# bing164/PL-VI-ORBSLAM3

Hardware: AMD Instinct MI355X
Metric: frames/sec ORB+LSD extract+match, 640×480 mono, 1/2/4/8 MI355X (higher is better)
Workload: dtype u8; 1 GPU; C1+C2+C3: ORB extract (1000 feats, 1.2, 8 levels, FAST 20/7) || LSD+LBD (200 lines, scale 0.8, 2 octaves) as one HIP-stream schedule, then ORB kNN-2 + LineMatcher::match vs previous frame; batch=3072, width=640, height=480, parallelism=sequence-sharded x1, gather=False, inflight=2

## Files before the change

### include/plvi_frontend.h

```cpp
#ifndef PLVI_FRONTEND_H
#define PLVI_FRONTEND_H

#include <stddef.h>
#include <stdint.h>

#ifdef __cplusplus
extern "C" {
#endif

enum {
  PLVI_OK = 0,
  PLVI_E_EMPTY = -1,
  PLVI_E_BADARG = -2,
  PLVI_E_CAPACITY = -3,
  PLVI_E_HIP = -4,
  PLVI_E_OVERFLOW = -5,
  PLVI_E_SIZE = -6,
  PLVI_E_CAPTURE = -7,
};

enum {
  PLVI_COMPAT_GAUSS_ROUNDED = 1,
  PLVI_COMPAT_RESIZE_V_GENERIC = 2,
  PLVI_COMPAT_EXP_CV_TABLE = 4,
// ... 90 lines not shown
int plvi_lines_extract_batch(plvi_line_extractor* h, const uint8_t* d_frames, int n_frames, size_t frame_stride,
                             size_t row_stride, void* stream);
int plvi_lines_outputs(plvi_line_extractor* h, plvi_keyline** d_kl, uint8_t** d_desc, double** d_fn, int** d_count,
                       int* cap);
int plvi_lines_errors(plvi_line_extractor* h, int* frame_flags, int* any, void* stream);

int plvi_lines_pyramid_level(plvi_line_extractor* h, int frame, int level, uint8_t* dst, int* w, int* hgt);

int plvi_lines_scale_tables(plvi_line_extractor* h, float* scale, float* inv_scale, float* sigma2, float* inv_sigma2);

int plvi_lines_profile(plvi_line_extractor* h, int enable);
int plvi_lines_debug_stats(plvi_line_extractor* h, unsigned long long* d_stats);
int plvi_lines_debug_mw_stats(plvi_line_extractor* h, int* d_stats);
int plvi_lines_debug_planes(plvi_line_extractor* h, int frame, int octave, float* deg, double* modgrad, float* cs,
                            int* sw, int* sh);
int plvi_lines_debug_sobel(plvi_line_extractor* h, int frame, int octave, short* dxdy, int* w, int* hgt);
int plvi_lines_debug_raw_lines(plvi_line_extractor* h, int frame, int octave, float* out, int cap, int* n);
int plvi_lines_profile_read(plvi_line_extractor* h, float* stage_ms, int* runs);
int plvi_lines_kernel_timing(plvi_line_extractor* h, int enable);
int plvi_lines_kernel_timing_read(plvi_line_extractor* h, float* total_ms, int* launches);
int plvi_lines_kernel_timing_read_kind(plvi_line_extractor* h, int kind, float* total_ms, int* launches);


int plvi_hamming_knn2_batch(const uint8_t* d_q, const int* d_nq, int nq_cap, const uint8_t* d_t, const int* d_nt,
                            int nt_cap, int n_pairs, int* d_idx0, int* d_d0, int* d_idx1, int* d_d1, void* stream);

int plvi_hamming_knn2(const uint8_t* q, int nq, const uint8_t* t, int nt, int* idx0, int* d0, int* idx1, int* d1);

int plvi_line_match_nnr(const uint8_t* desc1, int n1, const uint8_t* desc2, int n2, float nnr, int* matches_12);

// ... 756 lines not shown
```

### pl-vi-orbslam3_amd/csrc/lines_kernels.hpp

```cpp
#include <hip/hip_runtime.h>

#include "block_prims.h"
#include "lines_device.h"
#include "plvi_common.h"
#include "plvi_math.h"
#include "std_sort.h"

namespace plvi {

constexpr double kNotdef = -1024.0;
constexpr float kNotdefF = -1024.0f;
constexpr double kD2R = 3.14159265358979323846 / 180;
constexpr double kPi = 3.14159265358979323846;
constexpr double kLog10Of11 = 0x1.0a98b6050c56fp+0;

__global__ __launch_bounds__(256) void lsd_half_kernel(const uint8_t* __restrict__ src, size_t s_frame, size_t s_row,
                                                       uint8_t* __restrict__ dst, int dw, int dh, size_t d_frame) {
    const int f = blockIdx.y;
    const int i = blockIdx.x * 256 + threadIdx.x;
    if (i >= dw * dh) return;
    const int y = i / dw, x = i % dw;
    const uint8_t* S0 = src + (size_t)f * s_frame + (size_t)(2 * y) * s_row;
    const uint8_t* S1 = S0 + s_row;
    const int s = S0[2 * x] + S0[2 * x + 1] + S1[2 * x] + S1[2 * x + 1];
// ... 183 lines not shown
__device__ __forceinline__ void vm_drain() { __builtin_amdgcn_s_waitcnt(0); }

__device__ __forceinline__ bool used_get(const GrowCtx& g, int x, int y) {
    const bool inwin = y < g.wbb + g.RB;
    const int yy = inwin ? y : g.wbb;
    unsigned v = g.bits[(yy & (g.RB - 1)) * g.wpr + (x >> 5)];
    if (__builtin_expect(!inwin, 0)) v = gload_l2(g.gbits + (size_t)y * g.wpr + (x >> 5));
    return y < g.ys || ((v >> (x & 31)) & 1u);
}
__device__ __forceinline__ void used_set(const GrowCtx& g, int x, int y) {
    const unsigned b = 1u << (x & 31);
    if (__builtin_expect(y < g.wbb + g.RB, 1))
        __atomic_fetch_or(&g.bits[(y & (g.RB - 1)) * g.wpr + (x >> 5)], b, __ATOMIC_RELAXED);
    else __hip_atomic_fetch_or(g.gbits + (size_t)y * g.wpr + (x >> 5), b, __ATOMIC_RELAXED, __HIP_MEMORY_SCOPE_AGENT);
}
__device__ __forceinline__ void used_set_chunk(const GrowCtx& g, int xb, int y, unsigned long long mask, int lane) {
    const unsigned w = lane == 0 ? (unsigned)mask : (unsigned)(mask >> 32);
    if (lane < 2 && w) __atomic_fetch_or(&g.bits[(y & (g.RB - 1)) * g.wpr + (xb >> 5) + lane], w, __ATOMIC_RELAXED);
    __builtin_amdgcn_wave_barrier();
    __builtin_amdgcn_fence(__ATOMIC_ACQ_REL, "wavefront");
}
__device__ __forceinline__ unsigned q_get(const GrowCtx& g, int i) {
    if (__builtin_expect(i < g.QL, 1)) return g.qlds[i];
    return gload_l2(g.qglob + (i - g.QL));
}
__device__ __forceinline__ void q_put(const GrowCtx& g, int i, unsigned v) {
    if (__builtin_expect(i < g.QL, 1)) g.qlds[i] = v;
    else gstore_l2(g.qglob + (i - g.QL), v);
}
__device__ __forceinline__ float deg_at(const GrowCtx& g, int x, int y) {
    if (g.R == 0) return g.P[(size_t)y * g.sw + x];
    const bool inwin = y < g.wb + g.R;
    const int yy = inwin ? y : g.wb;
    float v = g.win[(yy & (g.R - 1)) * g.sw + x];
    if (__builtin_expect(!inwin, 0)) v = g.P[(size_t)y * g.sw + x];
    return v;
// ... 43 lines not shown
        }
    }
    for (; i < n; i += 64) {
        const int row = r0 + i / g.sw, x = i % g.sw;
        g.win[(row & (g.R - 1)) * g.sw + x] = src[i];
    }
}
__device__ __forceinline__ void bits_load_rows(const GrowCtx& g, int r0, int r1, int lane) {
    const int nw = (r1 - r0) * g.wpr;
    for (int k = lane; k < nw; k += 64) {
        const int row = r0 + k / g.wpr, w = k % g.wpr;
        g.bits[(row & (g.RB - 1)) * g.wpr + w] = gload_l2(g.gbits + (size_t)row * g.wpr + w);
    }
}

#ifndef PLVI_GROW_SETPRIO
#define PLVI_GROW_SETPRIO 3
#endif
#ifndef PLVI_GROW_OCT1_PRIO
#define PLVI_GROW_OCT1_PRIO PLVI_GROW_SETPRIO
#endif

#ifndef PLVI_GROW_WPE
#define PLVI_GROW_WPE 8
#endif
#ifndef PLVI_GROW_WG_WAVES
#define PLVI_GROW_WG_WAVES 4
#endif
constexpr int kGrowWaves = PLVI_GROW_WG_WAVES;

__device__ __forceinline__ void grow_wave_sync() {
    __builtin_amdgcn_fence(__ATOMIC_RELEASE, "wavefront");
    __builtin_amdgcn_wave_barrier();
    __builtin_amdgcn_fence(__ATOMIC_ACQUIRE, "wavefront");
    __builtin_amdgcn_sched_barrier(0);
}

constexpr int kGrowRB = 64, kGrowQL = 256;

template <bool STATS, bool FIXED, bool LOOP = false>
__global__ __launch_bounds__(64 * kGrowWaves, PLVI_GROW_WPE) void lsd_grow_kernel(const LineOctDev* __restrict__ octs,
                                                      const float* __restrict__ pix,
                                                      const double* __restrict__ modgrad,
                                                      const float2* __restrict__ pixcs,
                                                      unsigned* __restrict__ gbits_all, size_t gbits_frame,
                                                      unsigned* __restrict__ qspill, size_t qspill_frame,
                                                      double prec, LsdRegion* __restrict__ regs, unsigned* __restrict__ regpts,
                                                      size_t regpts_frame, int* __restrict__ nlines,
                                                      int* __restrict__ err, int R, int RB, int QL, int nOct,
                                                      int oBase, int oCount, unsigned long long* __restrict__ stats,
                                                      int nf, int ldsWave, int wpw) {
    extern __shared__ __align__(16) unsigned lds_all[];
    __builtin_amdgcn_s_setprio(PLVI_GROW_SETPRIO);
    const int wv = __builtin_amdgcn_readfirstlane((int)(threadIdx.x >> 6));
    const int ntask = nf * oCount, tstride = LOOP ? (int)gridDim.x * wpw : ntask;
    for (int task0 = blockIdx.x * wpw + wv; task0 < ntask; task0 += tstride) {
    const int task = __builtin_amdgcn_readfirstlane(task0);
    const int o = oBase + task / nf, f = task - (o - oBase) * nf;
    if (PLVI_GROW_OCT1_PRIO != PLVI_GROW_SETPRIO && o > 0) __builtin_amdgcn_s_setprio(PLVI_GROW_OCT1_PRIO);
    lds_u32* lds_w = (lds_u32*)lds_all + wv * (ldsWave >> 2);
// ... 3 lines not shown
    GrowCtx g;
    if (FIXED) {
        R = 0;
        RB = kGrowRB;
        QL = kGrowQL;
    }
    g.sw = sw; g.sh = sh; g.R = R; g.RB = RB; g.QL = QL;
    g.wpr = (sw + 31) >> 5;
    g.P = pix + od.soff + (size_t)f * od.splane;
    const float2* SC = pixcs + od.soff + (size_t)f * od.splane;
    LsdRegion* outR = regs + (size_t)(f * nOct + o) * kLsdRawCap;
    unsigned* outP = regpts + (size_t)(f * nOct + o) * regpts_frame;
    int npts = 0;
    g.gbits = gbits_all + (size_t)(f * nOct + o) * gbits_frame;
    g.qglob = qspill + (size_t)(f * nOct + o) * qspill_frame;
    g.bits = lds_w;
    g.qlds = g.bits + RB * g.wpr;
    g.win = (lds_f32*)(g.qlds + QL);
    g.wb = 0;
    g.wbb = 0;
    g.ys = 0;
    for (int i = lane; i < sh * g.wpr; i += 64) g.gbits[i] = 0u;
    for (int i = lane; i < RB * g.wpr; i += 64) g.bits[i] = 0u;
    if (R) win_load_rows(g, 0, min(R, sh), lane);
    vm_drain();
    grow_wave_sync();
    int nout = 0;
    bool overflow = false;
    const float pdeg = (float)(prec / kD2R);
    const int min_reg = od.min_reg_size;
    const int bp = lane / 9, bk = lane % 9;
    const int kdx = bk % 3 - 1, kdy = bk / 3 - 1;
    const unsigned long long below = (1ull << lane) - 1ull;
    unsigned long long s_setup = 0, s_round = 0, s_rect = 0, n_seed = 0, n_block = 0, n_round = 0, n_rpt = 0,
                       n_commit = 0;
    unsigned long long s_ph[4] = {0, 0, 0, 0};
    unsigned long long s_scan = 0, s_seed = 0, s_init = 0;
    unsigned long long n_far = 0, n_spill = 0;
    constexpr bool do_stats = STATS;
    const unsigned long long t_begin = do_stats ? __builtin_amdgcn_s_memtime() : 0;
    unsigned long long t_mark = t_begin;
    const unsigned long long t_real0 = do_stats ? __builtin_amdgcn_s_memrealtime() : 0;
    const int half = R / 2, halfb = RB / 2;
    auto chunk_load = [&](int cy, int cxb, float* v) {
        const int x = cxb + lane, xm = max(x - 1, 0), xx = min(x, sw - 1), xp = min(x + 1, sw - 1);
        const float* r0 = g.P + (size_t)cy * sw;
        const float* r1 = r0 + sw;
        v[0] = r0[xx]; v[1] = r0[xm]; v[2] = r0[xp];
        v[3] = r1[xm]; v[4] = r1[xx]; v[5] = r1[xp];
    };
    auto chunk_next = [&](int& cy, int& cxb) {
        if (cxb + 64 < sw - 1) {
            cxb += 64;
        } else {
            cxb = 0;
            ++cy;
        }
    };
    float nv[6], nv2[6];
    int py2 = 0, px2 = 0;
    chunk_load(0, 0, nv);
    chunk_next(py2, px2);
    if (py2 < sh - 1) chunk_load(py2, px2, nv2);
    if (do_stats) s_init = __builtin_amdgcn_s_memtime() - t_begin;
    for (int y = 0; y < sh - 1; ++y) {
        bool slid = false;
        while (R && y >= g.wb + half && g.wb + R < sh) {
            const int r0 = g.wb + R, r1 = min(sh, r0 + half);
            win_load_rows(g, r0, r1, lane);
            g.wb += r1 - r0;
            slid = true;
        }
        while (y >= g.wbb + halfb && g.wbb + RB < sh) {
            const int r0 = g.wbb + RB, r1 = min(sh, r0 + halfb);
            bits_load_rows(g, r0, r1, lane);
            g.wbb += r1 - r0;
            slid = true;
        }
        if (slid) {
            vm_drain();
            grow_wave_sync();
        }
        g.ys = y;
        for (int xb = 0; xb < sw - 1; xb += 64) {
            if (do_stats) t_mark = __builtin_amdgcn_s_memtime();
            float cv[6];
#pragma unroll
            for (int k = 0; k < 6; ++k) {
                cv[k] = nv[k];
                nv[k] = nv2[k];
            }
            chunk_next(py2, px2);
            if (py2 < sh - 1) chunk_load(py2, px2, nv2);
            const int x = xb + lane;
            bool cand = false, grow = false;
            if (x < sw - 1) {
                const float d0 = cv[0];
                cand = d0 != kNotdefF && !used_get(g, x, y);
                if (cand)
                    grow = (x > 0 && is_aligned_fast(cv[1], d0, pdeg, prec)) || is_aligned_fast(cv[2], d0, pdeg, prec) ||
                           (x > 0 && is_aligned_fast(cv[3], d0, pdeg, prec)) || is_aligned_fast(cv[4], d0, pdeg, prec) ||
                           is_aligned_fast(cv[5], d0, pdeg, prec);
            }
            unsigned long long m = __ballot(cand);
            if (do_stats) s_scan += __builtin_amdgcn_s_memtime() - t_mark;
            if (!m) continue;
            const unsigned long long gm = __ballot(grow);
            unsigned long long pend = m & ~gm;
            m &= gm;
            while (m) {
                const int b = __ffsll((long long)m) - 1;
                m &= m - 1;
                const int sx = xb + b;
                if (do_stats) t_mark = __builtin_amdgcn_s_memtime();
                const unsigned long long before = pend & ((1ull << b) - 1ull);
                if (before) {
                    used_set_chunk(g, xb, y, before, lane);
                    pend &= ~before;
                }
                if (used_get(g, sx, y)) continue;
                float reg_deg = readlane_f(cv[0], b);
                float sumdx = 0.f, sumdy = 0.f;
                if (lane == 0) {
                    used_set(g, sx, y);
                    g.qlds[0] = (unsigned)sx | ((unsigned)y << 16);
                }
                grow_wave_sync();
                if (do_stats) {
                    n_seed++;
                    s_seed += __builtin_amdgcn_s_memtime() - t_mark;
                }
                int reg_size = 1;
                for (int i = 0; i < reg_size;) {
                    const unsigned long long t0 = do_stats ? __builtin_amdgcn_s_memtime() : 0;
                    const int nb = min(7, reg_size - i);
                    const bool active = lane < 9 * nb;
                    unsigned pv;
                    if (i + 7 <= g.QL) {
                        const unsigned v = g.qlds[i + (active ? bp : 0)];
                        pv = active ? v : 0u;
                    } else {
                        pv = active ? q_get(g, i + bp) : 0u;
                    }
                    const int px = (int)(pv & 0xffffu), py = (int)(pv >> 16);
                    const int nx = px + kdx, ny = py + kdy;
                    const bool valid = active && nx >= 0 && nx < sw && ny >= y && ny < sh;
                    float deg = kNotdefF, cc = 0.f, ss = 0.f;
                    if (valid) {
                        const float2 cs2 = SC[(size_t)ny * sw + nx];
                        deg = deg_at(g, nx, ny);
                        cc = cs2.x;
                        ss = cs2.y;
                    }
                    if (i == 0) {
                        double ds, dc;
                        plvi_sincos((double)reg_deg * kD2R, &ds, &dc);
                        sumdx = (float)dc;
                        sumdy = (float)ds;
                    }
                    unsigned long long dup = 0;
                    for (int p2 = 0; p2 < nb - 1; ++p2) {
                        const unsigned q2 = (unsigned)readlane_i((int)pv, 9 * p2);
                        const int ddx = nx - (int)(q2 & 0xffffu) + 1, ddy = ny - (int)(q2 >> 16) + 1;
                        const bool hit = p2 < bp && (unsigned)ddx <= 2u && (unsigned)ddy <= 2u;
                        const unsigned long long hm = 0ull - (unsigned long long)hit;
                        dup |= (1ull << ((9 * p2 + ddy * 3 + ddx) & 63)) & hm;
                    }
                    unsigned long long t1 = 0;
                    if (do_stats) {
// ... 75 lines not shown
                    i += nb;
                }
                if (reg_size < min_reg) continue;
                const unsigned long long tr0 = do_stats ? __builtin_amdgcn_s_memtime() : 0;
                if (do_stats) n_rpt += reg_size;
                if (nout < kLsdRawCap) {
                    for (int j = lane; j < reg_size; j += 64) outP[npts + j] = q_get(g, j);
                    if (lane == 0) outR[nout] = LsdRegion{npts, reg_size, (double)reg_deg * kD2R};
                    npts += reg_size;
                    ++nout;
                } else {
                    overflow = true;
                }
                if (do_stats) s_rect += __builtin_amdgcn_s_memtime() - tr0;
            }
            if (pend) used_set_chunk(g, xb, y, pend, lane);
        }
    }
    if (lane == 0) {
        nlines[f * nOct + o] = nout;
        if (overflow) atomicOr(err + f, 4);
    }
    if (do_stats && lane == 0) {
        unsigned long long* S = stats + (size_t)(f * nOct + o) * 24;
        S[0] = __builtin_amdgcn_s_memtime() - t_begin;
        S[1] = s_setup; S[2] = s_round; S[3] = s_rect; S[4] = n_seed;
        S[5] = n_block; S[6] = n_round; S[7] = n_rpt; S[8] = n_commit;
        S[9] = s_ph[0]; S[10] = s_ph[1]; S[11] = s_ph[2]; S[12] = s_ph[3];
        S[13] = s_scan; S[14] = s_seed; S[15] = s_init;
        S[16] = __builtin_amdgcn_s_getreg((31 << 11) | 4);
        S[17] = __builtin_amdgcn_s_getreg((15 << 11) | 20);
// ... 715 lines not shown
```

### pl-vi-orbslam3_amd/csrc/lines_pipeline.hip

```cpp
#include <hip/hip_runtime.h>

#include <algorithm>
#include <cmath>
#include <cstdlib>
#include <cstring>
#include <memory>
#include <vector>

#include "lines_device.h"
#include "lines_kernels.hpp"
#include "lsd_grow_mw.hpp"
#include "plvi_common.h"

extern "C" int plvi_orb_internal_blur_event(plvi_orb_extractor* h, hipEvent_t ev);
extern "C" int plvi_orb_internal_stage_event(plvi_orb_extractor* h, int stage, hipEvent_t ev);

namespace plvi {

static inline int lround_h(float v) { return (int)lrintf(v); }
static inline int lround_h(double v) { return (int)lrint(v); }
static inline int lfloor_h(float v) { int i = (int)v; return i - (i > v); }

static double cv_exp64f(double x) {
    const double a0s = .9670371139572337719125840413672004409288e-2;
// ... 23 lines not shown
        sum += t;
    }
    sum *= 2;
    sum += 1.0;
    const double mul1 = 1.0 / sum;
    for (int i = 0; i < n2; ++i) k[i] = k[n - 1 - i] = values[i] * mul1;
    k[n2] = 1.0 * mul1;
}

struct LinePipeline {
    plvi_line_params prm{};
    int W = 0, H = 0, Bcap = 0, device = 0, nOct = 0, fcap = 0;
    hipStream_t stream = nullptr;
    hipStream_t aux[2] = {nullptr, nullptr};
    hipEvent_t evSobelGo = nullptr;
    hipEvent_t evFork = nullptr, evPrep = nullptr, evSobel = nullptr, evOrb = nullptr, evCrit = nullptr,
               evBlur = nullptr, evGate = nullptr, evGrow2 = nullptr, evPair = nullptr;
    bool growAfterBlur = true, sobelWithGrow = false, growSplit = false;
    int sobelGate = -1;
    bool sobelAfterGrow = false;
    hipStream_t critStream = nullptr;
    hipStream_t crit2 = nullptr;
    hipStream_t octStream = nullptr;
    int orbAfterPrep = 1;
    std::vector<LineOctDev> oct;
    std::vector<float> scaleF, invScaleF;
    double SCALE = 0.8, prec = 0, rho = 0, min_length = 0;
    double gk[7]{};
    int lbdTaps[3] = {14, 62, 104};
    DevBuf d_oct, d_tabs, octImg, pix, modg, seedcs, gbits, qspill, regs, regpts, rawLines, nlines, klTmp, klOut, fnOut, cntOut, descOut, lbdBlur,
        lbdG, err, staging, mwOwn, mwSlot, mwGrow, sortPos;
    size_t qspillFrame = 0, gbitsFrame = 0, lbdPlaneTotal = 0;
    int lastFrames = 0;
    static constexpr int kStages = 5, kRing = 512;
    bool prof = false;
    int profRuns = 0;
    std::vector<hipEvent_t> evs;

    static constexpr int kKRing = 4096;
    bool ktime = false;
    int kn = 0;
    std::vector<hipEvent_t> kev;
    std::vector<hipEvent_t> kevS[3];
    int knS[3] = {0, 0, 0};
    int ktiming(int on) {
// ... 35 lines not shown
            PLVI_CHECK(hipEventSynchronize(kev[2 * i + 1]));
            float t = 0.f;
            PLVI_CHECK(hipEventElapsedTime(&t, kev[2 * i], kev[2 * i + 1]));
            tot += t;
        }
        if (total_ms) *total_ms = tot;
        if (launches) *launches = kn;
        return PLVI_OK;
    }

    ~LinePipeline() {
        for (auto e : kev) (void)hipEventDestroy(e);
        for (auto& v : kevS)
            for (auto e : v) (void)hipEventDestroy(e);
        for (auto e : evs) (void)hipEventDestroy(e);
        for (auto e : {evFork, evPrep, evSobel, evOrb, evCrit, evBlur, evGate, evGrow2, evPair, evSobelGo})
            if (e) (void)hipEventDestroy(e);
        if (critStream) (void)hipStreamDestroy(critStream);
        if (crit2) (void)hipStreamDestroy(crit2);
        if (octStream) (void)hipStreamDestroy(octStream);
        for (auto a : aux)
            if (a) (void)hipStreamDestroy(a);
        if (stream) (void)hipStreamDestroy(stream);
    }

    int init(const plvi_line_params* p, int width, int height, int max_batch, int dev) {
        if (!p || width <= 0 || height <= 0 || max_batch <= 0) return PLVI_E_BADARG;
        if (p->refine != 0 || p->extractor != 0) return PLVI_E_BADARG;
        if (p->nlevels <= 0 || p->nlevels > kLineMaxOct || p->nfeatures < 0) return PLVI_E_BADARG;
        prm = *p;
        W = width; H = height; Bcap = max_batch; device = dev; nOct = p->nlevels;
// ... 12 lines not shown
            const bool orbHigh = !e4 || atoi(e4) != 0;
            for (int a = 0; a < 2; ++a)
                PLVI_CHECK(hipStreamCreateWithPriority(&aux[a], hipStreamNonBlocking,
                                                       prio ? (a == 0 && orbHigh ? greatest : least) : 0));
            const char* e5 = getenv("PLVI_SOBEL_WITH_GROW");
            sobelWithGrow = !e5 || atoi(e5) != 0;
            if (const char* e7 = getenv("PLVI_SOBEL_GATE")) sobelGate = std::min(5, std::max(-1, atoi(e7)));
            if (const char* e8 = getenv("PLVI_SOBEL_AFTER_GROW")) sobelAfterGrow = atoi(e8) != 0;
            if (prio) PLVI_CHECK(hipStreamCreateWithPriority(&critStream, hipStreamNonBlocking, greatest));
            const char* e6 = getenv("PLVI_GROW_SPLIT");
            growSplit = e6 && atoi(e6) != 0;
            if (prio && growSplit)
                PLVI_CHECK(hipStreamCreateWithPriority(&crit2, hipStreamNonBlocking, greatest));
            PLVI_CHECK(hipStreamCreateWithFlags(&octStream, hipStreamNonBlocking));
        }
        for (auto* e : {&evFork, &evPrep, &evSobel, &evOrb, &evCrit, &evBlur, &evGate, &evGrow2, &evPair, &evSobelGo})
            PLVI_CHECK(hipEventCreateWithFlags(e, hipEventDisableTiming));
        fcap = p->nfeatures > 0 ? p->nfeatures : kKlCap;
        SCALE = (double)p->lsd_scale;
        if (!(SCALE > 0) || SCALE > 1) return PLVI_E_BADARG;
        const double ANG_TH = 22.5, QUANT = 2.0, SIGMA_SCALE = 0.6;
        prec = M_PI * ANG_TH / 180;
        const double pp = ANG_TH / 180;
        rho = QUANT / std::sin(prec);
        min_length = 0.025 * std::min(W, H);
        const double sigma = (SCALE < 1) ? (SIGMA_SCALE / SCALE) : SIGMA_SCALE;
        const unsigned hk = (unsigned)std::ceil(sigma * std::sqrt(2 * 3.0 * std::log(10.0)));
        if (SCALE != 1 && 1 + 2 * hk != 7) return PLVI_E_BADARG;
        gauss_kernel_f64(7, sigma, gk, (p->compat & PLVI_COMPAT_EXP_CV_TABLE) != 0);
        if (SCALE == 1) gk[0] = gk[1] = gk[2] = 0.0, gk[3] = 1.0;
        lbdTaps[0] = 14;
// ... 150 lines not shown
            while (growR * 2 <= 1024 && fixed + perRow * growR * 2 <= budget) growR *= 2;
        }
        if (const char* e = getenv("PLVI_GROW_RD")) growR = atoi(e);
        if (growR < 0 || (growR & (growR - 1)) || growR == 1 || growR > 1024) return PLVI_E_BADARG;
        growSmem = (fixed + perRow * growR + 15) & ~size_t(15);
        if (growSmem > 160 * 1024) return PLVI_E_BADARG;
        growWPW = (int)std::max<size_t>(1, std::min<size_t>(kGrowWaves, (160 * 1024) / growSmem));
        for (const void* k : {(const void*)lsd_grow_kernel<false, false>, (const void*)lsd_grow_kernel<true, false>,
                              (const void*)lsd_grow_kernel<false, true>, (const void*)lsd_grow_kernel<true, true>,
                              (const void*)lsd_grow_kernel<false, true, true>})
            PLVI_CHECK(hipFuncSetAttribute(k, hipFuncAttributeMaxDynamicSharedMemorySize, (int)(growSmem * growWPW)));
        mwMaxFrames = 256;
        if (const char* e = getenv("PLVI_GROW_MW")) mwMaxFrames = atoi(e);
        if (const char* e = getenv("PLVI_GROW_TPW")) growTPW = std::max(0, atoi(e));
        mwMaxFrames = std::min(mwMaxFrames, Bcap);
        if (mwMaxFrames > 0) {
            const size_t nwords = gbitsFrame;
            const size_t fixedMw = sizeof(MwCtl) + 8 * kMwLog +
                                   4 * (3 * nwords + (size_t)kMwWaves * kMwRB * wprMax + (size_t)kMwWaves * kMwGQ);
            const size_t ldsMax = 160 * 1024;
            mwSlots = fixedMw < ldsMax ? (int)std::min<size_t>(kMwMaxSlots, (ldsMax - fixedMw) / kMwSlotBytes) : 0;
            mwSmem = fixedMw + (size_t)mwSlots * kMwSlotBytes;
            if (mwSlots < 2 * kMwWaves) {
                mwMaxFrames = 0;
            } else {
                const size_t tasks = (size_t)mwMaxFrames * nOct;
                mwOwnTask = (size_t)kMwWaves * gbitsFrame;
                if (mwOwn.alloc(sizeof(unsigned) * mwOwnTask * tasks) ||
                    mwSlot.alloc(sizeof(unsigned) * (size_t)mwSlots * kMwSlotSpill * tasks) ||
                    mwGrow.alloc(sizeof(unsigned) * (size_t)kMwWaves * kMwGSpill * tasks))
                    return PLVI_E_HIP;
                PLVI_CHECK(hipMemset(mwOwn.p, 0, mwOwn.bytes));
                for (const void* k : {(const void*)lsd_grow_mw_kernel<kMwWaves, false>,
                                      (const void*)lsd_grow_mw_kernel<kMwWaves, true>})
                    PLVI_CHECK(hipFuncSetAttribute(k, hipFuncAttributeMaxDynamicSharedMemorySize, (int)mwSmem));
            }
        }
        return PLVI_OK;
    }
// ... 28 lines not shown
        for (int k = 0; k < kStages; ++k) ms[k] = 0.f;
        for (int r = 0; r < profRuns; ++r) {
            PLVI_CHECK(hipEventSynchronize(evs[(size_t)r * (kStages + 1) + kStages]));
            for (int k = 0; k < kStages; ++k) {
                float t = 0.f;
                PLVI_CHECK(hipEventElapsedTime(&t, evs[(size_t)r * (kStages + 1) + k],
                                               evs[(size_t)r * (kStages + 1) + k + 1]));
                ms[k] += t;
            }
        }
        if (runs) *runs = profRuns;
        return PLVI_OK;
    }

    void launch_prep(const uint8_t* d_frames, int nf, size_t frame_stride, size_t row_stride, hipStream_t st,
                     int lFirst = 0, int lEnd = -1) {
        const uint8_t* T = d_tabs.as<uint8_t>();
        if (lEnd < 0) lEnd = nOct;
        for (int l = 1; l < nOct && lFirst == 0; ++l) {
            const LineOctDev& d = oct[l];
            const uint8_t* s = l == 1 ? d_frames : octImg.as<uint8_t>() + oct[l - 1].off;
            const size_t sf = l == 1 ? frame_stride : (size_t)oct[l - 1].plane;
            const size_t sr = l == 1 ? row_stride : (size_t)oct[l - 1].w;
            hipLaunchKernelGGL(lsd_half_kernel, dim3((d.w * d.h + 255) / 256, nf), dim3(256), 0, st, s, sf, sr,
                               octImg.as<uint8_t>() + d.off, d.w, d.h, (size_t)d.plane);
        }
        if (lFirst == 0) mark(1, st);
        for (int l = lFirst; l < lEnd; ++l) {
            const LineOctDev& d = oct[l];
            const uint8_t* s = l == 0 ? d_frames : octImg.as<uint8_t>() + d.off;
            const size_t sf = l == 0 ? frame_stride : (size_t)d.plane;
            const size_t sr = l == 0 ? row_stride : (size_t)d.w;
            const bool kt = ktime && kn < kKRing;
            if (kt) (void)hipEventRecord(kev[2 * kn], st);
            const bool banded = nf <= kPrepBandMax;
            hipLaunchKernelGGL(lsd_prep_kernel, dim3(d.nstrips, nf, banded ? kPrepBands : 1), dim3(64), 0, st, s, sf,
                               sr, d.w, d.h, d.sw, d.sh, (const int4*)(T + d.tabStrips),
                               (const int4*)(T + (banded ? d.tabBandsK : d.tabBands1)), (const int*)(T + d.tabXofs),
                               (const float*)(T + d.tabXa), d.xmax, (const int*)(T + d.tabYrow),
                               (const float*)(T + d.tabYb), gk[0], gk[1], gk[2], gk[3], rho,
                               pix.as<float>() + d.soff, modg.as<double>() + d.soff, seedcs.as<float2>() + d.soff,
                               (size_t)d.splane);
            if (kt) {
                (void)hipEventRecord(kev[2 * kn + 1], st);
                ++kn;
            }
        }
        if (lEnd == nOct) mark(2, st);
    }

    void launch_grow(int nf, int oBase, int oCount, hipStream_t st) {
        if (nf <= mwMaxFrames) {
            auto mwK = mwStats ? lsd_grow_mw_kernel<kMwWaves, true> : lsd_grow_mw_kernel<kMwWaves, false>;
            hipLaunchKernelGGL(mwK, dim3(oCount * nf), dim3(kMwWaves * 64), mwSmem, st, d_oct.as<LineOctDev>(),
                               (const float*)pix.as<float>(), (const float2*)seedcs.as<float2>(),
                               mwOwn.as<unsigned>(), mwOwnTask, mwGrow.as<unsigned>(), mwSlot.as<unsigned>(),
                               qspill.as<unsigned>(), qspillFrame, prec, regs.as<LsdRegion>(), regpts.as<unsigned>(),
                               qspillFrame, nlines.as<int>(), err.as<int>(), mwSlots, nOct, oBase, oCount, mwStats, nf,
                               mwStats && PLVI_MW_DIAG ? mwEpoch.as<int>() : nullptr);
            return;
        }
        const bool fixedWin = growR == 0 && growRB == kGrowRB && growQL == kGrowQL;
        const int tpwWant = growTPW > 0 ? growTPW : (inSchedule && nf >= 2048 ? 2 : 1);
        const int tpw = tpwWant > 1 && !growStats && fixedWin ? tpwWant : 1;
        auto growK = growStats ? (fixedWin ? lsd_grow_kernel<true, true> : lsd_grow_kernel<true, false>)
                               : (fixedWin ? (tpw > 1 ? lsd_grow_kernel<false, true, true> : lsd_grow_kernel<false, true>)
                                           : lsd_grow_kernel<false, false>);
        const int waves = (oCount * nf + tpw - 1) / tpw;
        hipLaunchKernelGGL(growK, dim3((waves + growWPW - 1) / growWPW), dim3(64 * growWPW),
                           growSmem * growWPW, st, d_oct.as<LineOctDev>(),
                           (const float*)pix.as<float>(), (const double*)modg.as<double>(),
                           (const float2*)seedcs.as<float2>(), gbits.as<unsigned>(), gbitsFrame,
                           qspill.as<unsigned>(), qspillFrame, prec, regs.as<LsdRegion>(), regpts.as<unsigned>(),
                           qspillFrame, nlines.as<int>(), err.as<int>(), growR, growRB, growQL, nOct, oBase, oCount,
                           growStats, nf, (int)growSmem, growWPW);
    }
    void launch_rect(int nf, int oBase, int oCount, hipStream_t st) {
        const int bx = nf <= 16 ? 8 : nf < kRectLargeNf ? kRectLaneBlocks : kRectLaneBlocksLarge;
        auto rectK = nf <= kRectSmallNf ? lsd_rect_lanes_kernel<kRectUSmall> : lsd_rect_lanes_kernel<kRectU>;
        ktimeS(2, 0, st);
        hipLaunchKernelGGL(rectK, dim3(bx, nf, oCount), dim3(256), 0, st, d_oct.as<LineOctDev>(),
                           (const double*)modg.as<double>(), (const LsdRegion*)regs.as<LsdRegion>(),
                           (const unsigned*)regpts.as<unsigned>(), qspillFrame, (const int*)nlines.as<int>(), prec,
                           SCALE, rawLines.as<LsdLine>(), oBase, nOct, qspill.as<double>(), qspillFrame / 2,
                           (int)(qspillFrame / 2));
        ktimeS(2, 1, st);
    }
    void launch_grow_assemble(int nf, hipStream_t st, bool grown = false, bool rect0 = false) {
// ... 87 lines not shown
        float nnr;
        int *lscratch, *lm12, *lnm;
    };
    int run_with_orb(const uint8_t* d_frames, int nf, size_t frame_stride, size_t row_stride, hipStream_t st,
                     plvi_orb_extractor* orb, int lap0, int lap1, const StepMatch* sm = nullptr) {
        if (nf <= 0 || nf > Bcap) return PLVI_E_BADARG;
        if (!st) st = stream;
        lastFrames = nf;
        const bool p0 = prof;
        prof = false;
        inSchedule = true;
        hipStream_t crit = critStream ? critStream : st;
        PLVI_CHECK(hipEventRecord(evFork, st));
        if (crit != st) PLVI_CHECK(hipStreamWaitEvent(crit, evFork, 0));
        const bool octFirst = nf <= mwMaxFrames && nOct > 1 && octStream;
        launch_prep(d_frames, nf, frame_stride, row_stride, crit, 0, octFirst ? 1 : nOct);
        PLVI_CHECK(hipEventRecord(evPrep, crit));
        if (octFirst) {
            PLVI_CHECK(hipStreamWaitEvent(octStream, evPrep, 0));
            launch_prep(d_frames, nf, frame_stride, row_stride, octStream, 1, nOct);
            launch_grow(nf, 1, nOct - 1, octStream);
            launch_rect(nf, 1, nOct - 1, octStream);
            PLVI_CHECK(hipEventRecord(evGrow2, octStream));
        }
        hipEvent_t auxStart = (orbAfterPrep >= 2 || (orbAfterPrep == 1 && nf < 1024)) ? evPrep : evFork;
        PLVI_CHECK(hipStreamWaitEvent(aux[0], auxStart, 0));
        const bool waitBlur = growAfterBlur && nf >= 1024;
        const bool sobelLate = waitBlur && sobelGate >= 0;
        if (waitBlur) plvi_orb_internal_blur_event(orb, evBlur);
        if (sobelLate) plvi_orb_internal_stage_event(orb, sobelGate, evSobelGo);
        int rc = plvi_orb_extract_batch(orb, d_frames, nf, frame_stride, row_stride, lap0, lap1, aux[0]);
        if (waitBlur) plvi_orb_internal_blur_event(orb, nullptr);
        if (sobelLate) plvi_orb_internal_stage_event(orb, -1, nullptr);
        if (sm && !rc) {
            plvi_keypoint* kp = nullptr;
            uint8_t* de = nullptr;
            int *co = nullptr, *mo = nullptr, cap = 0;
            rc = plvi_orb_outputs(orb, &kp, &de, &co, &mo, &cap);
            if (!rc)
                rc = plvi_hamming_knn2_batch(de + (size_t)cap * 32, co + 1, cap, de, co, cap, nf - 1, sm->idx0, sm->d0,
                                             sm->idx1, sm->d1, aux[0]);
        }
        PLVI_CHECK(hipEventRecord(evOrb, aux[0]));
        const bool split = waitBlur && growSplit && nOct == 2 && crit2 && !rc;
        hipStream_t gate = split ? crit2 : crit;
        if (split) {
            launch_grow(nf, 0, 1, crit);
            PLVI_CHECK(hipStreamWaitEvent(crit2, evPrep, 0));
        }
        if (waitBlur && !rc) PLVI_CHECK(hipStreamWaitEvent(gate, evBlur, 0));
        PLVI_CHECK(hipEventRecord(evGate, gate));
        const bool sobelAfter = sobelAfterGrow && waitBlur;
        if (!sobelAfter) {
            PLVI_CHECK(hipStreamWaitEvent(aux[1], sobelLate ? evSobelGo : sobelWithGrow ? evGate : auxStart, 0));
            if (!rc) rc = launch_sobel(d_frames, nf, frame_stride, row_stride, aux[1]);
            PLVI_CHECK(hipEventRecord(evSobel, aux[1]));
        }
        if (split) {
            launch_grow(nf, 1, 1, crit2);
            PLVI_CHECK(hipEventRecord(evGrow2, crit2));
            PLVI_CHECK(hipStreamWaitEvent(crit, evGrow2, 0));
        }
        if (octFirst) {
// ... 250 lines not shown
                                       float* cs, int* sw, int* sh) {
    if (!h || octave < 0 || octave >= h->p().nOct || frame < 0 || frame >= h->p().Bcap) return PLVI_E_BADARG;
    LinePipeline& P = h->p();
    PLVI_CHECK(hipSetDevice(P.device));
    const plvi::LineOctDev& d = P.oct[octave];
    const size_t n = (size_t)d.splane, o = (size_t)d.soff + (size_t)frame * n;
    if (sw) *sw = d.sw;
    if (sh) *sh = d.sh;
    PLVI_CHECK(hipDeviceSynchronize());
    if (deg) PLVI_CHECK(hipMemcpy(deg, P.pix.as<float>() + o, n * sizeof(float), hipMemcpyDeviceToHost));
    if (modgrad) PLVI_CHECK(hipMemcpy(modgrad, P.modg.as<double>() + o, n * sizeof(double), hipMemcpyDeviceToHost));
    if (cs) PLVI_CHECK(hipMemcpy(cs, P.seedcs.as<float2>() + o, n * sizeof(float2), hipMemcpyDeviceToHost));
    return PLVI_OK;
}

extern "C" int plvi_lines_debug_raw_lines(plvi_line_extractor* h, int frame, int octave, float* out, int cap, int* n) {
    if (!h || octave < 0 || octave >= h->p().nOct || frame < 0 || frame >= h->p().Bcap || cap < 0) return PLVI_E_BADARG;
    LinePipeline& P = h->p();
    PLVI_CHECK(hipSetDevice(P.device));
    PLVI_CHECK(hipDeviceSynchronize());
    const size_t task = (size_t)frame * P.nOct + octave;
    int cnt = 0;
    PLVI_CHECK(hipMemcpy(&cnt, P.nlines.as<int>() + task, sizeof(int), hipMemcpyDeviceToHost));
    cnt = std::min(cnt, plvi::kLsdRawCap);
    if (n) *n = cnt;
    if (cnt > cap) return PLVI_E_CAPACITY;
    if (out && cnt > 0)
        PLVI_CHECK(hipMemcpy(out, P.rawLines.as<plvi::LsdLine>() + task * plvi::kLsdRawCap,
                             sizeof(plvi::LsdLine) * cnt, hipMemcpyDeviceToHost));
    return PLVI_OK;
// ... 34 lines not shown
```

### pl-vi-orbslam3_amd/plvi/__init__.py

```python
import ctypes

import numpy as np

from ._abi import (HEADER_PATH, KEYLINE_DTYPE, KEYPOINT_DTYPE, LIB_PATH, PLVI_E_BADARG, PLVI_E_CAPACITY,
                   PLVI_E_CAPTURE, PLVI_E_EMPTY, PLVI_E_HIP, PLVI_E_OVERFLOW, PLVI_E_SIZE, PLVI_OK, DeviceBuffer,
                   PlviError, _check, _declare, _ptr, bound_runtime, c_int_p, c_void_pp, download,
                   exported_symbols, load, signatures)
from ._abi import (call as _call, out as _out, same_len as _same_len, status as _status, table as _table,
                   to_device as _to_device)

COMPAT_GAUSS_ROUNDED = 1
COMPAT_RESIZE_V_GENERIC = 2
COMPAT_EXP_CV_TABLE = 4


def _desc(a):
    return _table(a, np.uint8, 32)


def _sync():
    _call("plvi_device_synchronize")


class GridParams(ctypes.Structure):
# ... 400 lines not shown

    def kernel_timing_read(self, kind=0):
        return _timing_read("plvi_lines_kernel_timing_read_kind", self._h, kind)

    def pyramid_level(self, level, frame=0):
        return _sized_plane("plvi_lines_pyramid_level", self._h, frame, level, lambda h, w: (h, w), np.uint8)

    def debug_planes(self, level, frame=0):
        w, h = ctypes.c_int(), ctypes.c_int()
        _call("plvi_lines_debug_planes", self._h, frame, level, None, None, None, ctypes.byref(w), ctypes.byref(h))
        deg = np.zeros((h.value, w.value), np.float32)
        mg = np.zeros((h.value, w.value), np.float64)
        cs = np.zeros((h.value, w.value, 2), np.float32)
        _call("plvi_lines_debug_planes", self._h, frame, level, deg, mg, cs, None, None)
        return deg, mg, cs

    def debug_raw_lines(self, level, frame=0):
        n = ctypes.c_int()
        _call("plvi_lines_debug_raw_lines", self._h, frame, level, None, 1 << 30, ctypes.byref(n))
        lines = _out(n.value, 0, np.float32, 4)
        _call("plvi_lines_debug_raw_lines", self._h, frame, level, lines, n.value, ctypes.byref(n))
        return lines[:n.value].copy()

    def debug_sobel(self, level, frame=0):
        g = _sized_plane("plvi_lines_debug_sobel", self._h, frame, level, lambda h, w: (h, w, 2), np.int16)
        return g[..., 0].copy(), g[..., 1].copy()

    def scale_tables(self):
        tabs = [np.zeros(self.nlevels, np.float32) for _ in range(4)]
        _call("plvi_lines_scale_tables", self._h, *tabs)
# ... 1260 lines not shown
```

Before: 60760 frames/s.

## Precompute LSD seed grow/no-grow bitmasks in a parallel kernel before region growing

Adds a separate data-parallel kernel that computes, per pixel, whether an LSD seed candidate has an aligned neighbour, and packs the result into grow and no-grow bitmasks per 32-pixel word. The serial region-grow kernel then scans these masks word-wise instead of loading six neighbouring angles per pixel and testing alignment inline, so dense scanning work leaves the latency-bound grow loop. Used bits for non-growing candidates are set lazily when a seed is reached. The change adds an extra kernel launch, a mask buffer, a new event dependency before the grow stage, and a debug accessor. It only applies when the frame count exceeds the multi-wave grow threshold.

Result: no change. 60570 frames/s (-0.3%).

```diff
diff --git a/include/plvi_frontend.h b/include/plvi_frontend.h
--- a/include/plvi_frontend.h
+++ b/include/plvi_frontend.h
@@ -128,6 +128,8 @@
 int plvi_lines_debug_mw_stats(plvi_line_extractor* h, int* d_stats);
 int plvi_lines_debug_planes(plvi_line_extractor* h, int frame, int octave, float* deg, double* modgrad, float* cs,
                             int* sw, int* sh);
+int plvi_lines_debug_seed_masks(plvi_line_extractor* h, int frame, int octave, unsigned* grow, unsigned* nogrow,
+                                int* wpr, int* rows);
 int plvi_lines_debug_sobel(plvi_line_extractor* h, int frame, int octave, short* dxdy, int* w, int* hgt);
 int plvi_lines_debug_raw_lines(plvi_line_extractor* h, int frame, int octave, float* out, int cap, int* n);
 int plvi_lines_profile_read(plvi_line_extractor* h, float* stage_ms, int* runs);
diff --git a/pl-vi-orbslam3_amd/csrc/lines_kernels.hpp b/pl-vi-orbslam3_amd/csrc/lines_kernels.hpp
--- a/pl-vi-orbslam3_amd/csrc/lines_kernels.hpp
+++ b/pl-vi-orbslam3_amd/csrc/lines_kernels.hpp
@@ -221,12 +221,6 @@
         __atomic_fetch_or(&g.bits[(y & (g.RB - 1)) * g.wpr + (x >> 5)], b, __ATOMIC_RELAXED);
     else __hip_atomic_fetch_or(g.gbits + (size_t)y * g.wpr + (x >> 5), b, __ATOMIC_RELAXED, __HIP_MEMORY_SCOPE_AGENT);
 }
-__device__ __forceinline__ void used_set_chunk(const GrowCtx& g, int xb, int y, unsigned long long mask, int lane) {
-    const unsigned w = lane == 0 ? (unsigned)mask : (unsigned)(mask >> 32);
-    if (lane < 2 && w) __atomic_fetch_or(&g.bits[(y & (g.RB - 1)) * g.wpr + (xb >> 5) + lane], w, __ATOMIC_RELAXED);
-    __builtin_amdgcn_wave_barrier();
-    __builtin_amdgcn_fence(__ATOMIC_ACQ_REL, "wavefront");
-}
 __device__ __forceinline__ unsigned q_get(const GrowCtx& g, int i) {
     if (__builtin_expect(i < g.QL, 1)) return g.qlds[i];
     return gload_l2(g.qglob + (i - g.QL));
@@ -300,6 +294,82 @@
     }
 }
 
+constexpr int kSeedMaskRows = 32;
+constexpr int kSeedMaskWaves = 4;
+constexpr int kSeedMaskChunks = 8;
+
+struct SeedMaskRow {
+    float c[kSeedMaskChunks];
+    float e;
+};
+
+__global__ __launch_bounds__(64 * kSeedMaskWaves) void lsd_seed_mask_kernel(const float* __restrict__ pix,
+                                                                           size_t p_frame, int sw, int sh,
+                                                                           double prec, uint2* __restrict__ masks,
+                                                                           size_t m_frame) {
+    constexpr int K = kSeedMaskChunks;
+    const int lane = threadIdx.x & 63, wv = threadIdx.x >> 6;
+    const int xg = blockIdx.x * 64 * K, f = blockIdx.y;
+    const int yA = (blockIdx.z * kSeedMaskWaves + wv) * kSeedMaskRows;
+    if (yA >= sh) return;
+    const int yB = min(yA + kSeedMaskRows, sh);
+    const float* P = pix + (size_t)f * p_frame;
+    uint2* M = masks + (size_t)f * m_frame;
+    const int wpr = (sw + 31) >> 5;
+    const float pdeg = (float)(prec / kD2R);
+    const int ex = lane == 0 ? xg - 1 : xg + 64 * K;
+    const bool eok = gridDim.x > 1 && lane < 2 && ex >= 0 && ex < sw;
+    auto row_load = [&](int y, SeedMaskRow& r) {
+#pragma unroll
+        for (int k = 0; k < K; ++k) r.c[k] = kNotdefF;
+        r.e = kNotdefF;
+        if (y < sh) {
+            const float* p = P + (size_t)y * sw;
+#pragma unroll
+            for (int k = 0; k < K; ++k)
+                if (xg + 64 * k + lane < sw) r.c[k] = p[xg + 64 * k + lane];
+            if (eok) r.e = p[ex];
+        }
+    };
+    auto left = [&](const SeedMaskRow& r, int k) {
+        const float l = __int_as_float(dpp_from_left(__float_as_int(r.c[k])));
+        const float edge = k > 0 ? readlane_f(r.c[k > 0 ? k - 1 : 0], 63) : readlane_f(r.e, 0);
+        return lane == 0 ? edge : l;
+    };
+    auto right = [&](const SeedMaskRow& r, int k) {
+        const float v = __int_as_float(dpp_from_right(__float_as_int(r.c[k])));
+        const float edge = k < K - 1 ? readlane_f(r.c[k < K - 1 ? k + 1 : k], 0) : readlane_f(r.e, 1);
+        return lane == 63 ? edge : v;
+    };
+    SeedMaskRow cur, nxt, pre;
+    row_load(yA, cur);
+    row_load(yA + 1, nxt);
+    for (int y = yA; y < yB; ++y) {
+        row_load(y + 2 <= yB ? y + 2 : sh, pre);
+        uint2 out = make_uint2(0u, 0u);
+#pragma unroll
+        for (int k = 0; k < K; ++k) {
+            if (xg + 64 * k >= sw) continue;
+            const int x = xg + 64 * k + lane;
+            const float c0 = cur.c[k];
+            const float l0 = left(cur, k), r0 = right(cur, k), l1 = left(nxt, k), r1 = right(nxt, k);
+            const bool D = x < sw - 1 && y < sh - 1 && c0 != kNotdefF;
+            bool G = false;
+            if (D)
+                G = (x > 0 && is_aligned_fast(l0, c0, pdeg, prec)) || is_aligned_fast(r0, c0, pdeg, prec) ||
+                    (x > 0 && is_aligned_fast(l1, c0, pdeg, prec)) || is_aligned_fast(nxt.c[k], c0, pdeg, prec) ||
+                    is_aligned_fast(r1, c0, pdeg, prec);
+            const unsigned long long gm = ballot(G), nm = ballot(D && !G);
+            if (lane == 2 * k) out = make_uint2((unsigned)gm, (unsigned)nm);
+            if (lane == 2 * k + 1) out = make_uint2((unsigned)(gm >> 32), (unsigned)(nm >> 32));
+        }
+        const int w = (xg >> 5) + lane;
+        if (lane < 2 * K && w < wpr) M[(size_t)y * wpr + w] = out;
+        cur = nxt;
+        nxt = pre;
+    }
+}
+
 #ifndef PLVI_GROW_SETPRIO
 #define PLVI_GROW_SETPRIO 3
 #endif
@@ -330,6 +400,7 @@
                                                       const double* __restrict__ modgrad,
                                                       const float2* __restrict__ pixcs,
                                                       unsigned* __restrict__ gbits_all, size_t gbits_frame,
+                                                      const uint2* __restrict__ seedmask,
                                                       unsigned* __restrict__ qspill, size_t qspill_frame,
                                                       double prec, LsdRegion* __restrict__ regs, unsigned* __restrict__ regpts,
                                                       size_t regpts_frame, int* __restrict__ nlines,
@@ -363,6 +434,7 @@
     int npts = 0;
     g.gbits = gbits_all + (size_t)(f * nOct + o) * gbits_frame;
     g.qglob = qspill + (size_t)(f * nOct + o) * qspill_frame;
+    const uint2* SM = seedmask + (size_t)(f * nOct + o) * gbits_frame;
     g.bits = lds_w;
     g.qlds = g.bits + RB * g.wpr;
     g.win = (lds_f32*)(g.qlds + QL);
@@ -391,26 +463,13 @@
     unsigned long long t_mark = t_begin;
     const unsigned long long t_real0 = do_stats ? __builtin_amdgcn_s_memrealtime() : 0;
     const int half = R / 2, halfb = RB / 2;
-    auto chunk_load = [&](int cy, int cxb, float* v) {
-        const int x = cxb + lane, xm = max(x - 1, 0), xx = min(x, sw - 1), xp = min(x + 1, sw - 1);
-        const float* r0 = g.P + (size_t)cy * sw;
-        const float* r1 = r0 + sw;
-        v[0] = r0[xx]; v[1] = r0[xm]; v[2] = r0[xp];
-        v[3] = r1[xm]; v[4] = r1[xx]; v[5] = r1[xp];
+    int my = 0, mw = 0;
+    auto mask_load = [&]() {
+        uint2 v = make_uint2(0u, 0u);
+        if (my < sh - 1 && mw + lane < g.wpr) v = SM[(size_t)my * g.wpr + mw + lane];
+        return v;
     };
-    auto chunk_next = [&](int& cy, int& cxb) {
-        if (cxb + 64 < sw - 1) {
-            cxb += 64;
-        } else {
-            cxb = 0;
-            ++cy;
-        }
-    };
-    float nv[6], nv2[6];
-    int py2 = 0, px2 = 0;
-    chunk_load(0, 0, nv);
-    chunk_next(py2, px2);
-    if (py2 < sh - 1) chunk_load(py2, px2, nv2);
+    uint2 nm = mask_load();
     if (do_stats) s_init = __builtin_amdgcn_s_memtime() - t_begin;
     for (int y = 0; y < sh - 1; ++y) {
         bool slid = false;
@@ -431,49 +490,60 @@
             grow_wave_sync();
         }
         g.ys = y;
-        for (int xb = 0; xb < sw - 1; xb += 64) {
+        for (int w0 = 0; w0 < g.wpr; w0 += 64) {
             if (do_stats) t_mark = __builtin_amdgcn_s_memtime();
-            float cv[6];
-#pragma unroll
-            for (int k = 0; k < 6; ++k) {
-                cv[k] = nv[k];
-                nv[k] = nv2[k];
-            }
-            chunk_next(py2, px2);
-            if (py2 < sh - 1) chunk_load(py2, px2, nv2);
-            const int x = xb + lane;
-            bool cand = false, grow = false;
-            if (x < sw - 1) {
-                const float d0 = cv[0];
-                cand = d0 != kNotdefF && !used_get(g, x, y);
-                if (cand)
-                    grow = (x > 0 && is_aligned_fast(cv[1], d0, pdeg, prec)) || is_aligned_fast(cv[2], d0, pdeg, prec) ||
-                           (x > 0 && is_aligned_fast(cv[3], d0, pdeg, prec)) || is_aligned_fast(cv[4], d0, pdeg, prec) ||
-                           is_aligned_fast(cv[5], d0, pdeg, prec);
-            }
-            unsigned long long m = __ballot(cand);
+            const unsigned Gw = nm.x;
+            unsigned Nw = nm.y;
+            if (mw + 64 < g.wpr) {
+                mw += 64;
+            } else {
+                mw = 0;
+                ++my;
+            }
+            nm = mask_load();
+            const bool none = __ballot(Gw != 0u) == 0ull;
             if (do_stats) s_scan += __builtin_amdgcn_s_memtime() - t_mark;
-            if (!m) continue;
-            const unsigned long long gm = __ballot(grow);
-            unsigned long long pend = m & ~gm;
-            m &= gm;
-            while (m) {
-                const int b = __ffsll((long long)m) - 1;
-                m &= m - 1;
-                const int sx = xb + b;
+            if (none) continue;
+            lds_u32* brow = g.bits + (y & (g.RB - 1)) * g.wpr + min(w0 + lane, g.wpr - 1);
+            const int x0 = (w0 + lane) << 5;
+            int cbit = -1;
+            float cang = kNotdefF;
+            const float* Prow = g.P + (size_t)y * sw + x0;
+            while (true) {
                 if (do_stats) t_mark = __builtin_amdgcn_s_memtime();
-                const unsigned long long before = pend & ((1ull << b) - 1ull);
-                if (before) {
-                    used_set_chunk(g, xb, y, before, lane);
-                    pend &= ~before;
+                grow_wave_sync();
+                const unsigned avail = Gw & ~*brow;
+                const unsigned long long am = __ballot(avail != 0u);
+                if (!am) {
+                    if (do_stats) s_scan += __builtin_amdgcn_s_memtime() - t_mark;
+                    break;
                 }
-                if (used_get(g, sx, y)) continue;
-                float reg_deg = readlane_f(cv[0], b);
+                const int wl = __ffsll((long long)am) - 1;
+                const unsigned aw = (unsigned)readlane_i((int)avail, wl);
+                const int sb = __ffs((int)aw) - 1;
+                const int sx = ((w0 + wl) << 5) + sb;
+                const bool ahead = readlane_i(cbit, wl) == sb;
+                float reg_deg = readlane_f(cang, wl);
+                {
+                    const int nbit = __ffs((int)(lane == wl ? avail & (avail - 1u) : avail)) - 1;
+                    if (nbit != cbit) {
+                        cbit = nbit;
+                        if (nbit >= 0) cang = Prow[nbit];
+                    }
+                }
+                if (do_stats) {
+                    const unsigned long long t = __builtin_amdgcn_s_memtime();
+                    s_scan += t - t_mark;
+                    t_mark = t;
+                }
+                const int d = sx - x0;
+                const unsigned bm = d <= 0 ? 0u : d >= 32 ? ~0u : (1u << d) - 1u;
+                unsigned set = Nw & bm;
+                Nw &= ~bm;
+                if (d >= 0 && d < 32) set |= 1u << d;
+                if (set) __atomic_fetch_or(brow, set, __ATOMIC_RELAXED);
                 float sumdx = 0.f, sumdy = 0.f;
-                if (lane == 0) {
-                    used_set(g, sx, y);
-                    g.qlds[0] = (unsigned)sx | ((unsigned)y << 16);
-                }
+                if (lane == 0) g.qlds[0] = (unsigned)sx | ((unsigned)y << 16);
                 grow_wave_sync();
                 if (do_stats) {
                     n_seed++;
@@ -502,6 +572,11 @@
                         ss = cs2.y;
                     }
                     if (i == 0) {
+                        if (!ahead) {
+                            float dg = deg;
+                            asm volatile("" : "+v"(dg));
+                            reg_deg = readlane_f(dg, 4);
+                        }
                         double ds, dc;
                         plvi_sincos((double)reg_deg * kD2R, &ds, &dc);
                         sumdx = (float)dc;
@@ -607,7 +682,6 @@
                 }
                 if (do_stats) s_rect += __builtin_amdgcn_s_memtime() - tr0;
             }
-            if (pend) used_set_chunk(g, xb, y, pend, lane);
         }
     }
     if (lane == 0) {
diff --git a/pl-vi-orbslam3_amd/csrc/lines_pipeline.hip b/pl-vi-orbslam3_amd/csrc/lines_pipeline.hip
--- a/pl-vi-orbslam3_amd/csrc/lines_pipeline.hip
+++ b/pl-vi-orbslam3_amd/csrc/lines_pipeline.hip
@@ -61,6 +61,7 @@
     hipStream_t stream = nullptr;
     hipStream_t aux[2] = {nullptr, nullptr};
     hipEvent_t evSobelGo = nullptr;
+    hipEvent_t evMask = nullptr;
     hipEvent_t evFork = nullptr, evPrep = nullptr, evSobel = nullptr, evOrb = nullptr, evCrit = nullptr,
                evBlur = nullptr, evGate = nullptr, evGrow2 = nullptr, evPair = nullptr;
     bool growAfterBlur = true, sobelWithGrow = false, growSplit = false;
@@ -75,7 +76,7 @@
     double SCALE = 0.8, prec = 0, rho = 0, min_length = 0;
     double gk[7]{};
     int lbdTaps[3] = {14, 62, 104};
-    DevBuf d_oct, d_tabs, octImg, pix, modg, seedcs, gbits, qspill, regs, regpts, rawLines, nlines, klTmp, klOut, fnOut, cntOut, descOut, lbdBlur,
+    DevBuf d_oct, d_tabs, octImg, pix, modg, seedcs, gbits, seedMask, qspill, regs, regpts, rawLines, nlines, klTmp, klOut, fnOut, cntOut, descOut, lbdBlur,
         lbdG, err, staging, mwOwn, mwSlot, mwGrow, sortPos;
     size_t qspillFrame = 0, gbitsFrame = 0, lbdPlaneTotal = 0;
     int lastFrames = 0;
@@ -141,7 +142,7 @@
         for (auto& v : kevS)
             for (auto e : v) (void)hipEventDestroy(e);
         for (auto e : evs) (void)hipEventDestroy(e);
-        for (auto e : {evFork, evPrep, evSobel, evOrb, evCrit, evBlur, evGate, evGrow2, evPair, evSobelGo})
+        for (auto e : {evFork, evPrep, evSobel, evOrb, evCrit, evBlur, evGate, evGrow2, evPair, evSobelGo, evMask})
             if (e) (void)hipEventDestroy(e);
         if (critStream) (void)hipStreamDestroy(critStream);
         if (crit2) (void)hipStreamDestroy(crit2);
@@ -184,7 +185,7 @@
                 PLVI_CHECK(hipStreamCreateWithPriority(&crit2, hipStreamNonBlocking, greatest));
             PLVI_CHECK(hipStreamCreateWithFlags(&octStream, hipStreamNonBlocking));
         }
-        for (auto* e : {&evFork, &evPrep, &evSobel, &evOrb, &evCrit, &evBlur, &evGate, &evGrow2, &evPair, &evSobelGo})
+        for (auto* e : {&evFork, &evPrep, &evSobel, &evOrb, &evCrit, &evBlur, &evGate, &evGrow2, &evPair, &evSobelGo, &evMask})
             PLVI_CHECK(hipEventCreateWithFlags(e, hipEventDisableTiming));
         fcap = p->nfeatures > 0 ? p->nfeatures : kKlCap;
         SCALE = (double)p->lsd_scale;
@@ -365,6 +366,7 @@
         if (const char* e = getenv("PLVI_GROW_MW")) mwMaxFrames = atoi(e);
         if (const char* e = getenv("PLVI_GROW_TPW")) growTPW = std::max(0, atoi(e));
         mwMaxFrames = std::min(mwMaxFrames, Bcap);
+        if (Bcap > mwMaxFrames && seedMask.alloc(sizeof(uint2) * gbitsFrame * nOct * Bcap)) return PLVI_E_HIP;
         if (mwMaxFrames > 0) {
             const size_t nwords = gbitsFrame;
             const size_t fixedMw = sizeof(MwCtl) + 8 * kMwLog +
@@ -374,6 +376,7 @@
             mwSmem = fixedMw + (size_t)mwSlots * kMwSlotBytes;
             if (mwSlots < 2 * kMwWaves) {
                 mwMaxFrames = 0;
+                if (!seedMask.p && seedMask.alloc(sizeof(uint2) * gbitsFrame * nOct * Bcap)) return PLVI_E_HIP;
             } else {
                 const size_t tasks = (size_t)mwMaxFrames * nOct;
                 mwOwnTask = (size_t)kMwWaves * gbitsFrame;
@@ -432,7 +435,7 @@
     }
 
     void launch_prep(const uint8_t* d_frames, int nf, size_t frame_stride, size_t row_stride, hipStream_t st,
-                     int lFirst = 0, int lEnd = -1) {
+                     int lFirst = 0, int lEnd = -1, bool masks = true) {
         const uint8_t* T = d_tabs.as<uint8_t>();
         if (lEnd < 0) lEnd = nOct;
         for (int l = 1; l < nOct && lFirst == 0; ++l) {
@@ -463,8 +466,21 @@
                 (void)hipEventRecord(kev[2 * kn + 1], st);
                 ++kn;
             }
+            if (masks) launch_seed_masks(nf, st, l, l + 1);
         }
         if (lEnd == nOct) mark(2, st);
+    }
+    void launch_seed_masks(int nf, hipStream_t st, int lFirst, int lEnd) {
+        if (nf <= mwMaxFrames) return;
+        for (int l = lFirst; l < lEnd; ++l) {
+            const LineOctDev& d = oct[l];
+            hipLaunchKernelGGL(lsd_seed_mask_kernel,
+                               dim3((d.sw + 64 * kSeedMaskChunks - 1) / (64 * kSeedMaskChunks), nf,
+                                    (d.sh + kSeedMaskRows * kSeedMaskWaves - 1) / (kSeedMaskRows * kSeedMaskWaves)),
+                               dim3(64 * kSeedMaskWaves), 0, st, (const float*)pix.as<float>() + d.soff,
+                               (size_t)d.splane, d.sw, d.sh, prec, seedMask.as<uint2>() + (size_t)l * gbitsFrame,
+                               gbitsFrame * nOct);
+        }
     }
 
     void launch_grow(int nf, int oBase, int oCount, hipStream_t st) {
@@ -489,7 +505,8 @@
                            growSmem * growWPW, st, d_oct.as<LineOctDev>(),
                            (const float*)pix.as<float>(), (const double*)modg.as<double>(),
                            (const float2*)seedcs.as<float2>(), gbits.as<unsigned>(), gbitsFrame,
-                           qspill.as<unsigned>(), qspillFrame, prec, regs.as<LsdRegion>(), regpts.as<unsigned>(),
+                           (const uint2*)seedMask.as<uint2>(), qspill.as<unsigned>(), qspillFrame, prec,
+                           regs.as<LsdRegion>(), regpts.as<unsigned>(),
                            qspillFrame, nlines.as<int>(), err.as<int>(), growR, growRB, growQL, nOct, oBase, oCount,
                            growStats, nf, (int)growSmem, growWPW);
     }
@@ -607,8 +624,10 @@
         PLVI_CHECK(hipEventRecord(evFork, st));
         if (crit != st) PLVI_CHECK(hipStreamWaitEvent(crit, evFork, 0));
         const bool octFirst = nf <= mwMaxFrames && nOct > 1 && octStream;
-        launch_prep(d_frames, nf, frame_stride, row_stride, crit, 0, octFirst ? 1 : nOct);
+        launch_prep(d_frames, nf, frame_stride, row_stride, crit, 0, octFirst ? 1 : nOct, false);
         PLVI_CHECK(hipEventRecord(evPrep, crit));
+        launch_seed_masks(nf, crit, 0, nOct);
+        PLVI_CHECK(hipEventRecord(evMask, crit));
         if (octFirst) {
             PLVI_CHECK(hipStreamWaitEvent(octStream, evPrep, 0));
             launch_prep(d_frames, nf, frame_stride, row_stride, octStream, 1, nOct);
@@ -639,7 +658,7 @@
         hipStream_t gate = split ? crit2 : crit;
         if (split) {
             launch_grow(nf, 0, 1, crit);
-            PLVI_CHECK(hipStreamWaitEvent(crit2, evPrep, 0));
+            PLVI_CHECK(hipStreamWaitEvent(crit2, evMask, 0));
         }
         if (waitBlur && !rc) PLVI_CHECK(hipStreamWaitEvent(gate, evBlur, 0));
         PLVI_CHECK(hipEventRecord(evGate, gate));
@@ -920,6 +939,28 @@
     return PLVI_OK;
 }
 
+extern "C" int plvi_lines_debug_seed_masks(plvi_line_extractor* h, int frame, int octave, unsigned* grow,
+                                           unsigned* nogrow, int* wpr, int* rows) {
+    if (!h || octave < 0 || octave >= h->p().nOct || frame < 0 || frame >= h->p().Bcap) return PLVI_E_BADARG;
+    LinePipeline& P = h->p();
+    PLVI_CHECK(hipSetDevice(P.device));
+    const plvi::LineOctDev& d = P.oct[octave];
+    const int w = (d.sw + 31) / 32;
+    if (wpr) *wpr = w;
+    if (rows) *rows = d.sh;
+    if (!grow && !nogrow) return PLVI_OK;
+    if (!P.seedMask.p) return PLVI_E_BADARG;
+    PLVI_CHECK(hipDeviceSynchronize());
+    std::vector<uint2> m((size_t)w * d.sh);
+    PLVI_CHECK(hipMemcpy(m.data(), P.seedMask.as<uint2>() + ((size_t)frame * P.nOct + octave) * P.gbitsFrame,
+                         m.size() * sizeof(uint2), hipMemcpyDeviceToHost));
+    for (size_t i = 0; i < m.size(); ++i) {
+        if (grow) grow[i] = m[i].x;
+        if (nogrow) nogrow[i] = m[i].y;
+    }
+    return PLVI_OK;
+}
+
 extern "C" int plvi_lines_debug_raw_lines(plvi_line_extractor* h, int frame, int octave, float* out, int cap, int* n) {
     if (!h || octave < 0 || octave >= h->p().nOct || frame < 0 || frame >= h->p().Bcap || cap < 0) return PLVI_E_BADARG;
     LinePipeline& P = h->p();
diff --git a/pl-vi-orbslam3_amd/plvi/__init__.py b/pl-vi-orbslam3_amd/plvi/__init__.py
--- a/pl-vi-orbslam3_amd/plvi/__init__.py
+++ b/pl-vi-orbslam3_amd/plvi/__init__.py
@@ -438,6 +438,14 @@
         cs = np.zeros((h.value, w.value, 2), np.float32)
         _call("plvi_lines_debug_planes", self._h, frame, level, deg, mg, cs, None, None)
         return deg, mg, cs
+
+    def debug_seed_masks(self, level, frame=0):
+        w, h = ctypes.c_int(), ctypes.c_int()
+        _call("plvi_lines_debug_seed_masks", self._h, frame, level, None, None, ctypes.byref(w), ctypes.byref(h))
+        grow = np.zeros((h.value, w.value), np.uint32)
+        nogrow = np.zeros((h.value, w.value), np.uint32)
+        _call("plvi_lines_debug_seed_masks", self._h, frame, level, grow, nogrow, None, None)
+        return grow, nogrow
 
     def debug_raw_lines(self, level, frame=0):
         n = ctypes.c_int()
```
